# Lennart0HU/Master-Thesis-Deep-Reinforcement-Learning-DDPG-in-Home-Energy-Management

Hardware: NVIDIA B200
Metric: shems_LU1 env-steps/s (batched) (higher is better)
Workload: dtype f32/f64 mixed (Julia promotion rules)

## Files before the change

include/shems_b200.h:

```cpp
#ifndef SHEMS_B200_H
#define SHEMS_B200_H

#include <stdint.h>

#ifdef __cplusplus
extern "C" {
#endif

#define SHEMS_API __attribute__((visibility("default")))

enum {
  SHEMS_OK = 0,
  SHEMS_ERR_INVALID = -1,
  SHEMS_ERR_CUDA = -2,
  SHEMS_ERR_BOUNDS = -3,
  SHEMS_ERR_KEY = -4,
  SHEMS_ERR_STATE = -5
};

SHEMS_API const char* shems_last_error(void);
SHEMS_API int32_t shems_version(void);
SHEMS_API int64_t shems_env_kernel_launches(void);
SHEMS_API int32_t shems_device_count(void);

#define SHEMS_STATE_SIZE 9
#define SHEMS_ACTION_SIZE 2
#define SHEMS_TRACE_COLS 23
#define SHEMS_SERIES_COLS 8

enum {
  SHEMS_S_SOC_B = 0, SHEMS_S_SOC_EV, SHEMS_S_C_EV, SHEMS_S_D_E, SHEMS_S_G_E,
  SHEMS_S_P_BUY, SHEMS_S_H_COS, SHEMS_S_H_SIN, SHEMS_S_SEASON
};

enum {
  SHEMS_COL_SOC_EV = 0,
  SHEMS_COL_H_COUNTDOWN,
  SHEMS_COL_ELECTKWH,
  SHEMS_COL_PV_GENERATION,
  SHEMS_COL_P_BUY,
  SHEMS_COL_HOUR_COS,
  SHEMS_COL_HOUR_SIN,
  SHEMS_COL_SEASON
};

enum {
  SHEMS_T_INDEX = 0, SHEMS_T_C_EV, SHEMS_T_EV_TARGET, SHEMS_T_EV, SHEMS_T_SOC_EV,
  SHEMS_T_REWARD, SHEMS_T_PROFIT, SHEMS_T_DISCOMFORT, SHEMS_T_PENALTY, SHEMS_T_PV_DE,
  SHEMS_T_B_DE, SHEMS_T_GR_DE, SHEMS_T_PV_B, SHEMS_T_PV_GR, SHEMS_T_PV_EV, SHEMS_T_B_EV,
  SHEMS_T_GR_EV, SHEMS_T_EX_EV, SHEMS_T_GR_B, SHEMS_T_B_GR, SHEMS_T_B, SHEMS_T_B_TARGET,
  SHEMS_T_SOC_B
};

typedef struct ShemsParams {
  float pv_eta;
  float b_eta;
  float b_soc_min;
  float b_soc_max;
  double b_rate_max;
  float b_loss;
  float ev_soc_min;
  float ev_soc_max;
  float ev_rate_max;
  float penalty_weight;
  double sell_discount;
  double discomfort_weight_ev;
  double disc_pot;
  double penalty_weight_f64;
  int32_t penalty_in_f64;
  int32_t reward_form;
} ShemsParams;

SHEMS_API int32_t shems_params_for_charger(int32_t charger_id, ShemsParams* out);
enum { SHEMS_ENV_LU1 = 0, SHEMS_ENV_LU7 = 1, SHEMS_ENV_LU1_INPUT0607 = 2 };
SHEMS_API int32_t shems_params_for_env(int32_t env_variant, int32_t charger_id, ShemsParams* out);

SHEMS_API int32_t shems_series_from_csv(const char* path, float* series_out, int32_t capacity, int32_t* nrows_out);

typedef struct ShemsEnv ShemsEnv;

SHEMS_API int32_t shems_create(const ShemsParams* params, const float* series_host,
                               int32_t nrows, int32_t maxsteps, int64_t n_envs,
                               int32_t device, ShemsEnv** out);
SHEMS_API int32_t shems_create_groups(const ShemsParams* params, int32_t n_groups, const int64_t* group_sizes, const float* series_host,
                                      int32_t series_per_group, int32_t nrows, int32_t maxsteps, int32_t device, ShemsEnv** out);
SHEMS_API int32_t shems_destroy(ShemsEnv* env);
SHEMS_API int32_t shems_set_stream(ShemsEnv* env, void* cuda_stream);
SHEMS_API int32_t shems_sync(ShemsEnv* env);

enum { SHEMS_RESET_DETERMINISTIC = 0, SHEMS_RESET_HOST_DRAWS = 1, SHEMS_RESET_DEVICE_PHILOX = 2 };
SHEMS_API int32_t shems_reset(ShemsEnv* env, int32_t mode, const int32_t* idx0_host,
                              const float* socb0_host, uint64_t seed, int64_t env_id_base);

SHEMS_API int32_t shems_step(ShemsEnv* env, const float* act_dev, int32_t track,
                             float* reward_dev, double* reward64_dev, float* obs_dev, double* trace_dev);

SHEMS_API int32_t shems_action_rule(ShemsEnv* env, float* bev_dev);
SHEMS_API int32_t shems_action_drl(ShemsEnv* env, const float* target_dev, float* bev_dev);
SHEMS_API int32_t shems_finished(const ShemsEnv* env, int32_t* out);

SHEMS_API int32_t shems_state_ptr(ShemsEnv* env, float** obs_dev , int32_t** idx_dev );
SHEMS_API int32_t shems_get_state(ShemsEnv* env, float* obs_host , int32_t* idx_host );
SHEMS_API int32_t shems_set_state(ShemsEnv* env, const float* obs_host , const int32_t* idx_host );
SHEMS_API int32_t shems_get_step(const ShemsEnv* env, int32_t* step);
SHEMS_API int64_t shems_num_envs(const ShemsEnv* env);
// ... 135 lines not shown
```

master-thesis-deep-reinforcement-learning-ddpg-in-home-energy-management_b200/_lib.py:

```python
import ctypes as C
import os

HERE = os.path.dirname(os.path.abspath(__file__))
LIB_PATH = os.environ.get("SHEMS_B200_LIB", os.path.join(HERE, "libshems_b200.so"))

OK, ERR_INVALID, ERR_CUDA, ERR_BOUNDS, ERR_KEY, ERR_STATE = 0, -1, -2, -3, -4, -5
RESET_DETERMINISTIC, RESET_HOST_DRAWS, RESET_DEVICE_PHILOX = 0, 1, 2
POLICY_RULE, POLICY_RANDOM, POLICY_TAPE = 0, 1, 2
ENV_LU1, ENV_LU7, ENV_LU1_INPUT0607 = 0, 1, 2
NET_ACTOR, NET_CRITIC, NET_ACTOR_TARGET, NET_CRITIC_TARGET, NET_ACTOR_BEST = 0, 1, 2, 3, 4
DP_HANDLE_BYTES = 192


class ShemsParams(C.Structure):
    _fields_ = [
        ("pv_eta", C.c_float), ("b_eta", C.c_float), ("b_soc_min", C.c_float), ("b_soc_max", C.c_float),
        ("b_rate_max", C.c_double), ("b_loss", C.c_float), ("ev_soc_min", C.c_float), ("ev_soc_max", C.c_float),
        ("ev_rate_max", C.c_float), ("penalty_weight", C.c_float), ("sell_discount", C.c_double),
        ("discomfort_weight_ev", C.c_double), ("disc_pot", C.c_double),
        ("penalty_weight_f64", C.c_double), ("penalty_in_f64", C.c_int32), ("reward_form", C.c_int32),
    ]


class DdpgParams(C.Structure):
    _fields_ = [
        ("state_size", C.c_int32), ("action_size", C.c_int32), ("l1", C.c_int32), ("l2", C.c_int32),
        ("batch", C.c_int32), ("gamma", C.c_float), ("tau", C.c_float), ("lr_actor", C.c_float),
        ("lr_critic", C.c_float), ("adam_beta1", C.c_double), ("adam_beta2", C.c_double), ("adam_eps", C.c_double),
        ("act_lo", C.c_float * 2), ("act_hi", C.c_float * 2), ("use_tensor_cores", C.c_int32), ("population", C.c_int32),
    ]


class ShemsRolloutArgs(C.Structure):
    _fields_ = [
        ("policy", C.c_int32), ("n_steps", C.c_int32), ("seed", C.c_uint64), ("env_id_base", C.c_int64),
        ("tape_dev", C.c_void_p), ("ep_return_dev", C.c_void_p), ("replay", C.c_void_p), ("trace_dev", C.c_void_p),
        ("obs_traj_dev", C.c_void_p), ("reward_traj_dev", C.c_void_p), ("tape_unscaled", C.c_int32),
    ]


EXPLOIT_MAX_GROUPS = 16


class DdpgExploitParams(C.Structure):
    _fields_ = [
        ("frac", C.c_double), ("factor_lo", C.c_float), ("factor_hi", C.c_float), ("keys", C.c_int32), ("round", C.c_uint32),
        ("seed", C.c_uint64), ("n_groups", C.c_int32), ("group_start", C.c_int32 * (EXPLOIT_MAX_GROUPS + 1)),
    ]


class ShemsError(RuntimeError):
    def __init__(self, code, msg):
        super().__init__(f"[{code}] {msg}")
        self.code = code


class ShemsBoundsError(ShemsError, IndexError):
    """Julia BoundsError of next_state! (shems_LU1.jl:266-268)."""


class ShemsKeyError(ShemsError, KeyError):
    """Julia KeyError of capacities[charger_id] (shems_LU1.jl:95)."""


VP, PF, PI, PD = C.c_void_p, C.POINTER(C.c_float), C.POINTER(C.c_int32), C.POINTER(C.c_double)
I32, I64, U64, F32 = C.c_int32, C.c_int64, C.c_uint64, C.c_float

SIGNATURES = {
    "shems_last_error": (C.c_char_p, []),
    "shems_version": (I32, []),
    "shems_device_count": (I32, []),
    "shems_env_kernel_launches": (I64, []),
    "shems_params_for_charger": (I32, [I32, C.POINTER(ShemsParams)]),
    "shems_params_for_env": (I32, [I32, I32, C.POINTER(ShemsParams)]),
    "shems_series_from_csv": (I32, [C.c_char_p, PF, I32, PI]),
    "shems_create": (I32, [C.POINTER(ShemsParams), PF, I32, I32, I64, I32, C.POINTER(VP)]),
    "shems_create_groups": (I32, [C.POINTER(ShemsParams), I32, C.POINTER(I64), PF, I32, I32, I32, I32, C.POINTER(VP)]),
    "shems_destroy": (I32, [VP]),
    "shems_set_stream": (I32, [VP, VP]),
    "shems_sync": (I32, [VP]),
    "shems_reset": (I32, [VP, I32, PI, PF, U64, I64]),
    "shems_step": (I32, [VP, VP, I32, VP, VP, VP, VP]),
    "shems_action_rule": (I32, [VP, VP]),
    "shems_action_drl": (I32, [VP, VP, VP]),
    "shems_finished": (I32, [VP, PI]),
    "shems_state_ptr": (I32, [VP, C.POINTER(VP), C.POINTER(VP)]),
    "shems_get_state": (I32, [VP, PF, PI]),
    "shems_set_state": (I32, [VP, PF, PI]),
    "shems_get_step": (I32, [VP, PI]),
    "shems_num_envs": (I64, [VP]),
    "shems_num_rows": (I32, [VP]),
    "shems_rollout": (I32, [VP, C.POINTER(ShemsRolloutArgs)]),
    "replay_create": (I32, [I64, I32, C.POINTER(VP)]),
    "replay_destroy": (I32, [VP]),
    "replay_set_stream": (I32, [VP, VP]),
    "replay_length": (I64, [VP]),
    "replay_capacity": (I64, [VP]),
    "replay_series_count": (I32, [VP]),
    "replay_push": (I32, [VP, VP, VP, VP, VP, VP, I64]),
    "replay_push_groups": (I32, [C.POINTER(VP), I32, VP, VP, VP, VP, VP, I64]),
    "replay_sample": (I32, [VP, I32, PI, U64, VP, VP, VP, VP, VP]),
    "replay_minmax": (I32, [VP, I64, PI, U64, PF, PF]),
    "replay_get": (I32, [VP, PF, PF, PF, PF, PF]),
    "ddpg_default_params": (I32, [C.POINTER(DdpgParams)]),
    "ddpg_create": (I32, [C.POINTER(DdpgParams), I32, C.POINTER(VP)]),
    "ddpg_destroy": (I32, [VP]),
    "ddpg_set_stream": (I32, [VP, VP]),
    "ddpg_sync": (I32, [VP]),
    "ddpg_set_fused": (I32, [VP, I32]),
    "ddpg_init": (I32, [VP, U64]),
    "ddpg_set_layer": (I32, [VP, I32, I32, PF, PF]),
    "ddpg_get_layer": (I32, [VP, I32, I32, PF, PF]),
    "ddpg_get_grad": (I32, [VP, I32, I32, PF, PF]),
    "ddpg_num_params": (I64, [VP, I32]),
    "ddpg_set_norm": (I32, [VP, PF, PF]),
    "ddpg_act": (I32, [VP, VP, I64, F32, U64, I64, I64, VP, VP, VP]),
    "ddpg_act_soa": (I32, [VP, VP, I64, F32, U64, I64, I64, VP, VP, VP]),
    "ddpg_act_ou": (I32, [VP, VP, I64, F32, F32, F32, F32, VP, U64, I64, I64, VP, VP, VP]),
    "ddpg_set_noise": (I32, [VP, I32, F32, F32, F32]),
    "ddpg_episode": (I32, [VP, VP, C.POINTER(VP), I32, I32, F32, U64, I32, I64, VP, VP]),
    "ddpg_update": (I32, [VP, VP, I32, PI, U64]),
    "ddpg_update_phase": (I32, [VP, VP, I32, PI, U64, F32]),
    "ddpg_update_batch": (I32, [VP, VP, VP, VP, VP, VP]),
    "ddpg_dp_export": (I32, [VP, VP]),
    "ddpg_dp_connect": (I32, [VP, I32, I32, VP]),
    "ddpg_dp_prepare": (I32, [VP, I64]),
    "ddpg_update_dp": (I32, [VP, VP, I32, PI, U64]),
    "ddpg_dp_status": (I32, [VP, PI]),
    "ddpg_get_losses": (I32, [VP, PF, PF]),
    "ddpg_select_learner": (I32, [VP, I32]),
    "ddpg_population": (I32, [VP]),
    "ddpg_update_population": (I32, [VP, C.POINTER(VP), I32, PI, C.POINTER(U64)]),
    "ddpg_set_hparams": (I32, [VP, F32, F32, F32, F32, F32]),
    "ddpg_get_hparams": (I32, [VP, PF, PF, PF, PF, PF]),
    "shems_tc_gemm": (I32, [VP, I64, I32, VP, I64, I32, VP, I64, I32, I32, I32, I32, VP, VP, I64, I32, VP, VP]),
    "ddpg_grad_buffer": (I32, [VP, C.POINTER(VP), C.POINTER(I64)]),
    "ddpg_rollout": (I32, [VP, VP, I32, F32, U64, I64, VP, VP, VP]),
    "ddpg_evaluate": (I32, [VP, VP, I32, I32, I64, VP, VP, VP]),
    "ddpg_keep_best": (I32, [VP, VP, I64, I32, VP]),
    "ddpg_get_best": (I32, [VP, PD, PI]),
    "ddpg_set_best": (I32, [VP, PD, PI]),
    "ddpg_exploit": (I32, [VP, VP, C.POINTER(DdpgExploitParams), VP]),
    "ddpg_state_floats": (I64, [VP]),
    "ddpg_get_state": (I32, [VP, PF, PD]),
    "ddpg_set_state": (I32, [VP, PF, PD]),
    "ddpg_get_ou_state": (I32, [VP, PF, C.POINTER(I64)]),
    "ddpg_set_ou_state": (I32, [VP, PF, I64]),
}

_lib = None


def lib():
    global _lib
    if _lib is None:
# ... 46 lines not shown
```

master-thesis-deep-reinforcement-learning-ddpg-in-home-energy-management_b200/csrc/common.h:

```cpp
#pragma once
#include <cuda_runtime.h>
#include <stdint.h>
#include <stdio.h>
#include <stdarg.h>
#include "../../include/shems_b200.h"
#include "ring.cuh"

void shems_set_error(const char* fmt, ...);

#define CUDA_TRY(expr)                                                                     \
  do {                                                                                     \
    cudaError_t _e = (expr);                                                               \
    if (_e != cudaSuccess) {                                                               \
      shems_set_error("%s:%d %s -> %s", __FILE__, __LINE__, #expr, cudaGetErrorString(_e)); \
      return SHEMS_ERR_CUDA;                                                               \
    }                                                                                      \
  } while (0)

#define REQUIRE(cond, code, ...)  \
  do {                            \
    if (!(cond)) {                \
      shems_set_error(__VA_ARGS__); \
      return (code);              \
    }                             \
  } while (0)

struct DeviceGuard {
  int prev = -1;
  bool ok = true;
  explicit DeviceGuard(int dev) {
    if (cudaGetDevice(&prev) != cudaSuccess) { ok = false; return; }
    if (prev != dev && cudaSetDevice(dev) != cudaSuccess) ok = false;
  }
  ~DeviceGuard() { if (prev >= 0) cudaSetDevice(prev); }
};
#define GUARD(dev)                                             \
  DeviceGuard _guard(dev);                                     \
  if (!_guard.ok) {                                            \
    cudaError_t _e = cudaGetLastError();                       \
    shems_set_error("cannot select CUDA device %d: %s", (dev), cudaGetErrorString(_e)); \
    return SHEMS_ERR_CUDA;                                     \
  }

struct DevParams {
  float pv_eta, b_eta, smin, smax, loss, evmin, evmax, evR, pw;
  float one_m_l;
  float one_m_l_e;
  float C;
  float span;
  float R_f;
  float R_dn, R_up;
  float smax95_up;
  double R, sell, dw, pot;
  double pw_d;
  int pen_f64, reward_form;
  int reward_mode;
  double eta_d, one_m_l_d, C_d, smax95;
  float r_eta_f, r_span_f;
  double r_eta_d, r_C_d;
  int fast_eta_f, fast_span_f;
  int fast_d;
  double span_d, r_span_d;
  int fast_all;
};

#define SHEMS_MAX_GROUPS 16

struct RingSeries {
  unsigned long long env_serial;
  int series;
  int nrows;
  float* rows;
};

struct ShemsReplay {
  int device;
  cudaStream_t stream;
  int64_t capacity, length, head;
  float* alloc;
  float* ring;
  int32_t* idx_scratch;
  int64_t idx_scratch_n;
  float* minmax_scratch;
  void* group_refs; int group_refs_n;
  RingSeries src[RING_MAX_SERIES];
  const float* src_ptrs[RING_MAX_SERIES];
  int n_src;
};

struct ShemsEnv {
  int device;
  cudaStream_t stream;
  DevParams dp;
  ShemsParams params;
  int32_t nrows, maxsteps;
  int64_t n;
  float4* series;
  float* obs;
  int32_t* idx;
  int32_t* d_maxidx;
  int32_t max_idx;
  int32_t* h_maxidx;
  cudaEvent_t ev_maxidx; bool max_pending;
  int32_t step;
  unsigned long long serial;
  bool was_reset;
  bool consistent;
  int32_t* scratch_i; float* scratch_f;
  int n_groups;
  DevParams gdp[SHEMS_MAX_GROUPS];
  float4* gseries[SHEMS_MAX_GROUPS];
  long long gstart[SHEMS_MAX_GROUPS + 1];
};

int replay_after_rollout(ShemsReplay* rp, int64_t n_written);
int replay_series_entry(ShemsReplay* rp, unsigned long long serial, int series, const float4* rows_dev, int nrows, cudaStream_t user,
                        int* entry);
int32_t ensure_rows(ShemsEnv* e, int64_t need);
```

master-thesis-deep-reinforcement-learning-ddpg-in-home-energy-management_b200/csrc/env.cu:

```cuda
#include <new>
#include <vector>
#include <string.h>
#include <math.h>
#include <stdlib.h>

#include "common.h"
#include "philox.cuh"
#include "shems_device.cuh"

static thread_local char g_err[512] = "";
void shems_set_error(const char* fmt, ...) {
  va_list ap;
  va_start(ap, fmt);
  vsnprintf(g_err, sizeof(g_err), fmt, ap);
  va_end(ap);
}
extern "C" const char* shems_last_error(void) { return g_err; }
extern "C" int32_t shems_version(void) { return 200; }
static long long g_env_launches = 0;
extern "C" int64_t shems_env_kernel_launches(void) { return __atomic_load_n(&g_env_launches, __ATOMIC_RELAXED); }
#define COUNT_LAUNCH() __atomic_add_fetch(&g_env_launches, 1, __ATOMIC_RELAXED)
extern "C" int32_t shems_device_count(void) {
  int n = 0;
  if (cudaGetDeviceCount(&n) != cudaSuccess) { cudaGetLastError(); return 0; }
// ... 371 lines not shown
                          const float* __restrict__ tape, int tape_unscaled, RolloutSinks S, long long n0, long long n1, int lockstep) {
  const long long n = n0 + (long long)blockIdx.x * blockDim.x + threadIdx.x;
  if (n >= n1) return;
  int idx = idx_arr[n];
  float Soc_b = obs[0 * N + n], Soc_ev = obs[1 * N + n];
  float c_ev, d_e, g_e, p_buy;
  { const Row8 r = load_row(series, idx); c_ev = r.cd; d_e = r.d_e; g_e = r.g_e; p_buy = r.p_buy; }
  double ret = 0.0;
  RingWalk ring{};
  if (S.ring) { long long slot = S.head + n; if (slot >= S.cap) slot -= S.cap; ring = ring_walk(S.ring, slot, N, S.cap); }
  const uint64_t id = (uint64_t)(env_id_base + n);
  auto step = [&](auto cls, int t, uint32_t w0, uint32_t w1) {
    constexpr int CLS = decltype(cls)::value;
    StepIn s;
    s.Soc_b = Soc_b; s.Soc_ev = Soc_ev; s.c_ev = c_ev; s.d_e = d_e; s.g_e = g_e; s.p_buy = p_buy;
    float B, EV, Bt, EVt, a_raw0, a_raw1;
    bool track_neg = false;
    if (POLICY == SHEMS_POLICY_RULE) {
      shems_action_rule<true>(P, s.Soc_b, s.Soc_ev, s.d_e, s.g_e, B, EV);
      Bt = 0.0f; EVt = 0.0f; a_raw0 = B; a_raw1 = EV; track_neg = true;
    } else {
      if (POLICY == SHEMS_POLICY_RANDOM) {
        a_raw0 = action_from_word(w0);
        a_raw1 = action_from_word(w1);
        Bt = (a_raw0 + 1.0f) * 0.5f;
        EVt = (a_raw1 + 1.0f) * 0.5f;
      } else {
        Bt = tape[((size_t)t * 2 + 0) * N + n];
        EVt = tape[((size_t)t * 2 + 1) * N + n];
        a_raw0 = Bt; a_raw1 = EVt;
        if (tape_unscaled) {
          Bt = (float)(((double)a_raw0 + 1.0) * 0.5);
          EVt = (float)(((double)a_raw1 + 1.0) * 0.5);
        }
      }
      shems_action_drl<true, CLS>(P, s.Soc_b, s.Soc_ev, s.c_ev, s.d_e, s.g_e, Bt, EVt, B, EV);
    }
    StepTrace tr;
    const StepOut o = shems_flows<false, true, CLS>(P, s, B, EV, EVt, track_neg, &tr);
    const Row8 nx = load_row(series, idx + 1);
    float Soc_ev_new = o.Soc_ev;
    if (nx.cd >= 0.0f && (CLS == ROW_ANY ? c_ev == -1.0f : row_noev<CLS>)) Soc_ev_new = nx.soc_ev;
    if (S.ring) {
      ring_store_compact(ring.q, Soc_b, Soc_ev, a_raw0, a_raw1, (float)o.reward, o.Soc_b, Soc_ev_new, S.src_entry, idx);
      ring_walk_next(ring);
    }
    if (S.reward_traj) S.reward_traj[(size_t)t * N + n] = (float)o.reward;
    Soc_b = o.Soc_b; Soc_ev = Soc_ev_new; c_ev = nx.cd; d_e = nx.d_e; g_e = nx.g_e; p_buy = nx.p_buy;
    idx += 1;
    ret += o.reward;
  };
  const unsigned mask = __activemask();
  if (lockstep && __all_sync(mask, idx == __shfl_sync(mask, idx, __ffs(mask) - 1))) {
    uint32_t rw[4] = {0u, 0u, 0u, 0u};
    for (int t = 0; t < T; ++t) {
      if (POLICY == SHEMS_POLICY_RANDOM) {
        const unsigned st_abs = (unsigned)(step0 + t);
        if ((st_abs & 1u) == 0u || t == 0) philox4x32_10(K, id, st_abs >> 1, STREAM_ACTION, rw);
        if (st_abs & 1u) { rw[0] = rw[2]; rw[1] = rw[3]; }
      }
      switch (row_class(P, c_ev, d_e, g_e)) {
        case ROW_A_NOEV: step(RowTag<ROW_A_NOEV>{}, t, rw[0], rw[1]); break;
        case ROW_B_NOEV: step(RowTag<ROW_B_NOEV>{}, t, rw[0], rw[1]); break;
        case ROW_A_EV: step(RowTag<ROW_A_EV>{}, t, rw[0], rw[1]); break;
        case ROW_B_EV: step(RowTag<ROW_B_EV>{}, t, rw[0], rw[1]); break;
        default: step(RowTag<ROW_ANY>{}, t, rw[0], rw[1]); break;
      }
    }
  } else {
    for (int t = POLICY == SHEMS_POLICY_RANDOM ? -(step0 & 1) : 0; t < T; t += 2) {
      uint32_t rw[4] = {0u, 0u, 0u, 0u};
      if (POLICY == SHEMS_POLICY_RANDOM) philox4x32_10(K, id, (unsigned)(step0 + t) >> 1, STREAM_ACTION, rw);
      if (t >= 0) step(RowTag<ROW_ANY>{}, t, rw[0], rw[1]);
      if (t + 1 < T) step(RowTag<ROW_ANY>{}, t + 1, rw[2], rw[3]);
    }
  }
  const Row8 r = load_row(series, idx);
  obs[0 * N + n] = Soc_b; obs[1 * N + n] = Soc_ev; obs[2 * N + n] = r.cd; obs[3 * N + n] = r.d_e; obs[4 * N + n] = r.g_e;
  obs[5 * N + n] = r.p_buy; obs[6 * N + n] = r.h_cos; obs[7 * N + n] = r.h_sin; obs[8 * N + n] = r.season;
  idx_arr[n] = idx;
  if (S.ep_return) S.ep_return[n] = ret;
}

static inline unsigned grid_for(long long n, int block) { return (unsigned)((n + block - 1) / block); }

static int rollout_min_blocks(int device, long long n, bool compact, bool lean) {
  static int forced = -1;
  if (forced < 0) { const char* ev = getenv("SHEMS_ROLLOUT_MIN_BLOCKS"); forced = ev ? atoi(ev) : 0; }
  if (forced == 6 || forced == 7 || forced == 8) return forced;
  if (compact) return lean ? 7 : 6;
  static int sms[64];
  if (device >= 0 && device < 64 && sms[device] == 0) {
    int v = 0;
    if (cudaDeviceGetAttribute(&v, cudaDevAttrMultiProcessorCount, device) != cudaSuccess || v <= 0) { cudaGetLastError(); v = 148; }
    sms[device] = v;
  }
  const int nsm = (device >= 0 && device < 64) ? sms[device] : 148;
  const double ctas = (double)((n + ROLLOUT_THREADS - 1) / ROLLOUT_THREADS);
  int best = ROLLOUT_MIN_BLOCKS; double best_cost = 1e300;
  for (int b = 6; b <= 8; ++b) {
    const double waves = ctas / ((double)nsm * b);
    const double full = floor(waves), frac = waves - full;
    const double last = frac > 0.0 ? (frac < 0.45 ? 0.45 : frac) : 0.0;
    const double penalty = b == 6 ? 1.0 : (b == 7 ? 1.015 : 1.03);
    const double cost = (full + last) * b * penalty;
    if (cost < best_cost - 1e-9) { best_cost = cost; best = b; }
  }
  return best;
}

static bool ring_compact_enabled() {
  const char* ev = getenv("SHEMS_RING_COMPACT");
  return !(ev && atoi(ev) == 0);
}

static bool rollout_lean_enabled() {
  const char* ev = getenv("SHEMS_ROLLOUT_LEAN");
  return !(ev && atoi(ev) == 0);
}

static bool rollout_lockstep_enabled() {
  const char* ev = getenv("SHEMS_ROLLOUT_LOCKSTEP");
  return !(ev && atoi(ev) == 0);
}

extern "C" int32_t shems_create_groups(const ShemsParams* params, int32_t n_groups, const int64_t* group_sizes, const float* series_host,
                                       int32_t series_per_group, int32_t nrows, int32_t maxsteps, int32_t device, ShemsEnv** out) {
  REQUIRE(params && series_host && out && group_sizes, SHEMS_ERR_INVALID, "shems_create: NULL argument");
  REQUIRE(n_groups >= 1 && n_groups <= SHEMS_MAX_GROUPS, SHEMS_ERR_INVALID, "shems_create: n_groups=%d (1..%d)", n_groups, SHEMS_MAX_GROUPS);
  int64_t n_envs = 0;
  for (int g = 0; g < n_groups; ++g) {
    REQUIRE(group_sizes[g] >= 1, SHEMS_ERR_INVALID, "shems_create: group_sizes[%d]=%lld", g, (long long)group_sizes[g]);
    n_envs += group_sizes[g];
  }
  REQUIRE(nrows >= 2 && maxsteps >= 1, SHEMS_ERR_INVALID, "shems_create: nrows=%d maxsteps=%d", nrows, maxsteps);
  REQUIRE(nrows - maxsteps >= 1, SHEMS_ERR_INVALID,
          "shems_create: nrows - maxsteps = %d < 1: rand(1:(nrow-maxsteps)) would be empty (shems_LU1.jl:225)", nrows - maxsteps);
  REQUIRE(shems_device_count() > 0, SHEMS_ERR_CUDA, "shems_create: no CUDA device (this library has no CPU fallback)");
  GUARD(device);
  ShemsEnv* e = new (std::nothrow) ShemsEnv();
  REQUIRE(e, SHEMS_ERR_INVALID, "shems_create: out of host memory");
  memset(e, 0, sizeof(*e));
  e->device = device; e->stream = 0; e->params = params[0]; e->dp = make_dev_params(params[0]);
  e->nrows = nrows; e->maxsteps = maxsteps; e->n = n_envs; e->max_idx = 1; e->consistent = true;
  e->n_groups = n_groups;
  static unsigned long long next_serial = 0;
  e->serial = __atomic_add_fetch(&next_serial, 1, __ATOMIC_RELAXED);
  const int n_series = series_per_group ? n_groups : 1;
  std::vector<float> rows((size_t)n_series * nrows * 8);
  for (int g = 0; g < n_series; ++g)
    for (int r = 0; r < nrows; ++r)
      for (int c = 0; c < 8; ++c) rows[((size_t)g * nrows + r) * 8 + c] = series_host[((size_t)g * 8 + c) * nrows + r];
  cudaError_t st = cudaSuccess;
  if ((st = cudaMalloc(&e->series, sizeof(float) * rows.size())) != cudaSuccess ||
      (st = cudaMalloc(&e->obs, sizeof(float) * 9 * (size_t)n_envs)) != cudaSuccess ||
      (st = cudaMalloc(&e->idx, sizeof(int32_t) * (size_t)n_envs)) != cudaSuccess ||
      (st = cudaMalloc(&e->d_maxidx, sizeof(int32_t))) != cudaSuccess ||
      (st = cudaMemcpy(e->series, rows.data(), sizeof(float) * rows.size(), cudaMemcpyHostToDevice)) != cudaSuccess ||
      (st = cudaMemset(e->obs, 0, sizeof(float) * 9 * (size_t)n_envs)) != cudaSuccess ||
      (st = cudaMemset(e->idx, 0, sizeof(int32_t) * (size_t)n_envs)) != cudaSuccess) {
    shems_set_error("shems_create: %s", cudaGetErrorString(st));
    shems_destroy(e);
    return SHEMS_ERR_CUDA;
  }
  if ((st = cudaMallocHost((void**)&e->h_maxidx, sizeof(int32_t))) != cudaSuccess ||
      (st = cudaEventCreateWithFlags(&e->ev_maxidx, cudaEventDisableTiming)) != cudaSuccess) {
    shems_set_error("shems_create: %s", cudaGetErrorString(st));
    shems_destroy(e);
    return SHEMS_ERR_CUDA;
  }
  for (int g = 0; g < n_groups; ++g) {
    e->gdp[g] = make_dev_params(params[g]);
    e->gseries[g] = e->series + (series_per_group ? (size_t)g * nrows * 2 : 0);
    e->gstart[g + 1] = e->gstart[g] + group_sizes[g];
  }
  *out = e;
  return SHEMS_OK;
}

extern "C" int32_t shems_create(const ShemsParams* params, const float* series_host, int32_t nrows, int32_t maxsteps,
                                int64_t n_envs, int32_t device, ShemsEnv** out) {
  REQUIRE(n_envs >= 1, SHEMS_ERR_INVALID, "shems_create: n_envs=%lld", (long long)n_envs);
  return shems_create_groups(params, 1, &n_envs, series_host, 0, nrows, maxsteps, device, out);
}

extern "C" int32_t shems_destroy(ShemsEnv* e) {
  if (!e) return SHEMS_OK;
  GUARD(e->device);
  cudaFree(e->series); cudaFree(e->obs); cudaFree(e->idx); cudaFree(e->d_maxidx); cudaFree(e->scratch_i); cudaFree(e->scratch_f);
  if (e->h_maxidx) cudaFreeHost(e->h_maxidx);
  if (e->ev_maxidx) cudaEventDestroy(e->ev_maxidx);
  delete e;
  return SHEMS_OK;
}

extern "C" int32_t shems_set_stream(ShemsEnv* e, void* s) {
  REQUIRE(e, SHEMS_ERR_INVALID, "shems_set_stream: NULL handle");
  e->stream = (cudaStream_t)s;
  return SHEMS_OK;
}
extern "C" int32_t shems_sync(ShemsEnv* e) {
  REQUIRE(e, SHEMS_ERR_INVALID, "shems_sync: NULL handle");
  GUARD(e->device);
  CUDA_TRY(cudaStreamSynchronize(e->stream));
  return SHEMS_OK;
}
extern "C" int64_t shems_num_envs(const ShemsEnv* e) { return e ? e->n : 0; }
extern "C" int32_t shems_num_rows(const ShemsEnv* e) { return e ? e->nrows : 0; }
extern "C" int32_t shems_get_step(const ShemsEnv* e, int32_t* step) {
  REQUIRE(e && step, SHEMS_ERR_INVALID, "shems_get_step: NULL argument");
  *step = e->step;
  return SHEMS_OK;
}
extern "C" int32_t shems_finished(const ShemsEnv* e, int32_t* out) {
  REQUIRE(e && out, SHEMS_ERR_INVALID, "shems_finished: NULL argument");
  *out = 0;
  return SHEMS_OK;
}

int32_t ensure_rows(ShemsEnv* e, int64_t need) {
  if ((int64_t)e->max_idx + need <= e->nrows) return 0;
  if (e->max_pending) {
    cudaEventSynchronize(e->ev_maxidx);
    e->max_idx = *e->h_maxidx + e->step;
    e->max_pending = false;
    if ((int64_t)e->max_idx + need <= e->nrows) return 0;
  }
  return e->max_idx;
}

extern "C" int32_t shems_reset(ShemsEnv* e, int32_t mode, const int32_t* idx0_host, const float* socb0_host, uint64_t seed,
                               int64_t env_id_base) {
  REQUIRE(e, SHEMS_ERR_INVALID, "shems_reset: NULL handle");
  REQUIRE(mode >= 0 && mode <= 2, SHEMS_ERR_INVALID, "shems_reset: unknown mode %d", mode);
  GUARD(e->device);
  const int hi = e->nrows - e->maxsteps;
  if (mode == SHEMS_RESET_HOST_DRAWS) {
    REQUIRE(idx0_host && socb0_host, SHEMS_ERR_INVALID, "shems_reset: HOST_DRAWS needs idx0_host and socb0_host");
    for (int64_t i = 0; i < e->n; ++i)
      REQUIRE(idx0_host[i] >= 1 && idx0_host[i] <= hi, SHEMS_ERR_INVALID, "shems_reset: idx0[%lld]=%d outside 1..%d", (long long)i,
              idx0_host[i], hi);
    if (!e->scratch_i) {
      CUDA_TRY(cudaMalloc(&e->scratch_i, sizeof(int32_t) * (size_t)e->n));
      CUDA_TRY(cudaMalloc(&e->scratch_f, sizeof(float) * (size_t)e->n));
    }
    CUDA_TRY(cudaMemcpyAsync(e->scratch_i, idx0_host, sizeof(int32_t) * (size_t)e->n, cudaMemcpyHostToDevice, e->stream));
    CUDA_TRY(cudaMemcpyAsync(e->scratch_f, socb0_host, sizeof(float) * (size_t)e->n, cudaMemcpyHostToDevice, e->stream));
  }
  CUDA_TRY(cudaMemsetAsync(e->d_maxidx, 0, sizeof(int32_t), e->stream));
  for (int g = 0; g < e->n_groups; ++g) {
    const long long n0 = e->gstart[g], n1 = e->gstart[g + 1];
    COUNT_LAUNCH();
    shems_reset_kernel<<<grid_for(n1 - n0, 256), 256, 0, e->stream>>>(e->gdp[g], e->gseries[g], e->nrows, e->maxsteps, e->n, mode, e->scratch_i,
                                                                     e->scratch_f, seed, env_id_base, e->obs, e->idx, e->d_maxidx, n0, n1);
  }
  CUDA_TRY(cudaGetLastError());
  if (mode == SHEMS_RESET_DETERMINISTIC) { e->max_idx = 1; e->max_pending = false; }
  else {
    CUDA_TRY(cudaMemcpyAsync(e->h_maxidx, e->d_maxidx, sizeof(int32_t), cudaMemcpyDeviceToHost, e->stream));
    CUDA_TRY(cudaEventRecord(e->ev_maxidx, e->stream));
    e->max_idx = hi; e->max_pending = true;
  }
  e->step = 0;
  e->was_reset = true;
  e->consistent = true;
  return SHEMS_OK;
}

extern "C" int32_t shems_step(ShemsEnv* e, const float* act_dev, int32_t track, float* reward_dev, double* reward64_dev, float* obs_dev,
                              double* trace_dev) {
  REQUIRE(e && act_dev, SHEMS_ERR_INVALID, "shems_step: NULL argument");
  REQUIRE(e->was_reset, SHEMS_ERR_STATE, "shems_step: reset! (or shems_set_state) must come first");
  if (ensure_rows(e, 1)) {
    shems_set_error("BoundsError: attempt to access %d-row series at row %d (next_state!, shems_LU1.jl:266-268)", e->nrows, e->max_idx + 1);
    return SHEMS_ERR_BOUNDS;
  }
  GUARD(e->device);
  const int tn = track < 0 ? 1 : 0;
#define LAUNCH_STEP(FS, TR)                                                                                                             \
  COUNT_LAUNCH();                                                                                                                       \
  if (!TR && e->gdp[g].fast_all)                                                                                                        \
    shems_step_kernel<FS, false, true><<<grid_for(n1 - n0, STEP_THREADS), STEP_THREADS, 0, e->stream>>>(                                   \
        e->gdp[g], e->gseries[g], e->n, e->obs, e->idx, act_dev, tn, reward_dev, reward64_dev, obs_dev, trace_dev, n0, n1);              \
  else                                                                                                                                  \
    shems_step_kernel<FS, TR, false><<<grid_for(n1 - n0, STEP_THREADS), STEP_THREADS, 0, e->stream>>>(                                     \
        e->gdp[g], e->gseries[g], e->n, e->obs, e->idx, act_dev, tn, reward_dev, reward64_dev, obs_dev, trace_dev, n0, n1)
  for (int g = 0; g < e->n_groups; ++g) {
    const long long n0 = e->gstart[g], n1 = e->gstart[g + 1];
    if (e->consistent) { if (trace_dev) { LAUNCH_STEP(true, true); } else { LAUNCH_STEP(true, false); } }
    else { if (trace_dev) { LAUNCH_STEP(false, true); } else { LAUNCH_STEP(false, false); } }
  }
#undef LAUNCH_STEP
  CUDA_TRY(cudaGetLastError());
  e->max_idx += 1;
  e->step += 1;
  e->consistent = true;
  return SHEMS_OK;
}

extern "C" int32_t shems_action_rule(ShemsEnv* e, float* bev_dev) {
  REQUIRE(e && bev_dev, SHEMS_ERR_INVALID, "shems_action_rule: NULL argument");
  GUARD(e->device);
  for (int g = 0; g < e->n_groups; ++g, COUNT_LAUNCH())
    shems_action_kernel<true><<<grid_for(e->gstart[g + 1] - e->gstart[g], 256), 256, 0, e->stream>>>(e->gdp[g], e->n, e->obs, nullptr, bev_dev,
                                                                                                    e->gstart[g], e->gstart[g + 1]);
  CUDA_TRY(cudaGetLastError());
  return SHEMS_OK;
}
extern "C" int32_t shems_action_drl(ShemsEnv* e, const float* target_dev, float* bev_dev) {
  REQUIRE(e && target_dev && bev_dev, SHEMS_ERR_INVALID, "shems_action_drl: NULL argument");
  GUARD(e->device);
  for (int g = 0; g < e->n_groups; ++g, COUNT_LAUNCH())
    shems_action_kernel<false><<<grid_for(e->gstart[g + 1] - e->gstart[g], 256), 256, 0, e->stream>>>(e->gdp[g], e->n, e->obs, target_dev, bev_dev,
                                                                                                     e->gstart[g], e->gstart[g + 1]);
  CUDA_TRY(cudaGetLastError());
  return SHEMS_OK;
}

extern "C" int32_t shems_state_ptr(ShemsEnv* e, float** obs_dev, int32_t** idx_dev) {
  REQUIRE(e, SHEMS_ERR_INVALID, "shems_state_ptr: NULL handle");
  if (obs_dev) *obs_dev = e->obs;
  if (idx_dev) *idx_dev = e->idx;
  return SHEMS_OK;
}
extern "C" int32_t shems_get_state(ShemsEnv* e, float* obs_host, int32_t* idx_host) {
  REQUIRE(e && obs_host, SHEMS_ERR_INVALID, "shems_get_state: NULL argument");
  GUARD(e->device);
  CUDA_TRY(cudaMemcpyAsync(obs_host, e->obs, sizeof(float) * 9 * (size_t)e->n, cudaMemcpyDeviceToHost, e->stream));
  if (idx_host) CUDA_TRY(cudaMemcpyAsync(idx_host, e->idx, sizeof(int32_t) * (size_t)e->n, cudaMemcpyDeviceToHost, e->stream));
  CUDA_TRY(cudaStreamSynchronize(e->stream));
  return SHEMS_OK;
}
extern "C" int32_t shems_set_state(ShemsEnv* e, const float* obs_host, const int32_t* idx_host) {
  REQUIRE(e && obs_host && idx_host, SHEMS_ERR_INVALID, "shems_set_state: NULL argument");
  GUARD(e->device);
  int32_t mx = 1;
  for (int64_t i = 0; i < e->n; ++i) {
    REQUIRE(idx_host[i] >= 1 && idx_host[i] <= e->nrows, SHEMS_ERR_INVALID, "shems_set_state: idx[%lld]=%d outside 1..%d", (long long)i,
            idx_host[i], e->nrows);
    mx = idx_host[i] > mx ? idx_host[i] : mx;
  }
  CUDA_TRY(cudaMemcpyAsync(e->obs, obs_host, sizeof(float) * 9 * (size_t)e->n, cudaMemcpyHostToDevice, e->stream));
  CUDA_TRY(cudaMemcpyAsync(e->idx, idx_host, sizeof(int32_t) * (size_t)e->n, cudaMemcpyHostToDevice, e->stream));
  CUDA_TRY(cudaStreamSynchronize(e->stream));
  e->max_idx = mx; e->max_pending = false;
  e->was_reset = true;
  e->consistent = false;
  return SHEMS_OK;
}

extern "C" int32_t shems_rollout(ShemsEnv* e, const ShemsRolloutArgs* a) {
  REQUIRE(e && a, SHEMS_ERR_INVALID, "shems_rollout: NULL argument");
  REQUIRE(e->was_reset, SHEMS_ERR_STATE, "shems_rollout: reset! must come first");
  REQUIRE(a->n_steps >= 1, SHEMS_ERR_INVALID, "shems_rollout: n_steps=%d", a->n_steps);
  REQUIRE(a->policy >= 0 && a->policy <= 2, SHEMS_ERR_INVALID, "shems_rollout: unknown policy %d", a->policy);
  REQUIRE(a->policy != SHEMS_POLICY_TAPE || a->tape_dev, SHEMS_ERR_INVALID, "shems_rollout: POLICY_TAPE needs tape_dev");
  REQUIRE(!(a->policy == SHEMS_POLICY_TAPE && a->replay && !a->tape_unscaled), SHEMS_ERR_INVALID,
          "shems_rollout: POLICY_TAPE with a replay sink needs tape_unscaled = 1 (actions in [-1,1], as remember() stores them)");
  if (ensure_rows(e, a->n_steps)) {
    shems_set_error("BoundsError: rollout of %d steps from row %d leaves the %d-row series (next_state!, shems_LU1.jl:266-268)", a->n_steps,
                    e->max_idx, e->nrows);
    return SHEMS_ERR_BOUNDS;
  }
  GUARD(e->device);
  RolloutSinks S;
  memset(&S, 0, sizeof(S));
  S.ep_return = a->ep_return_dev; S.trace = a->trace_dev; S.obs_traj = a->obs_traj_dev; S.reward_traj = a->reward_traj_dev;
  S.cap = 1;
  const int64_t total = (int64_t)a->n_steps * e->n;
  if (a->replay) {
    ShemsReplay* rp = a->replay;
    REQUIRE(rp->device == e->device, SHEMS_ERR_INVALID, "shems_rollout: replay lives on device %d, env on %d", rp->device, e->device);
    REQUIRE(total <= rp->capacity || rp->capacity % e->n == 0, SHEMS_ERR_INVALID,
            "shems_rollout: replay capacity %lld must hold n_steps*n_envs=%lld or be a multiple of n_envs=%lld", (long long)rp->capacity,
            (long long)total, (long long)e->n);
    REQUIRE(e->n <= rp->capacity, SHEMS_ERR_INVALID, "shems_rollout: replay capacity %lld < n_envs %lld", (long long)rp->capacity, (long long)e->n);
    S.ring = rp->ring; S.cap = rp->capacity; S.head = rp->head;
  }
#define LAUNCH_RO_F(POL, TR, MB, FA, CO)                                                                                            \
  shems_rollout_kernel<POL, TR, MB, FA, CO><<<grid_for(n1 - n0, ROLLOUT_THREADS), ROLLOUT_THREADS, 0, e->stream>>>(                      \
      e->gdp[g], e->gseries[g], e->n, e->obs, e->idx, a->n_steps, e->step, a->seed, a->env_id_base, a->tape_dev, a->tape_unscaled, S, n0, n1)
#define LAUNCH_RO_C(POL, TR, MB, FA)                                                                                                \
  do { if (compact) LAUNCH_RO_F(POL, TR, MB, FA, true); else LAUNCH_RO_F(POL, TR, MB, FA, false); } while (0)
#define LAUNCH_RO(POL, TR, MB)                                                                                                      \
  do { if (!TR && e->gdp[g].fast_all) LAUNCH_RO_C(POL, false, MB, true); else LAUNCH_RO_C(POL, TR, MB, false); } while (0)
#define LAUNCH_RO_MB(POL)                                                                                                           \
  do {                                                                                                                              \
    if (tr) LAUNCH_RO(POL, true, ROLLOUT_MIN_BLOCKS);                                                                               \
    else if (mb == 7) LAUNCH_RO(POL, false, 7);                                                                                     \
    else if (mb == 8) LAUNCH_RO(POL, false, 8);                                                                                     \
    else LAUNCH_RO(POL, false, ROLLOUT_MIN_BLOCKS);                                                                                 \
  } while (0)
#define LAUNCH_LEAN(POL, MB)                                                                                                        \
  shems_rollout_lean_kernel<POL, MB><<<grid_for(n1 - n0, ROLLOUT_THREADS), ROLLOUT_THREADS, 0, e->stream>>>(                           \
      e->gdp[g], e->gseries[g], e->n, e->obs, e->idx, a->n_steps, e->step, keys, a->env_id_base, a->tape_dev, a->tape_unscaled, S, n0, n1, \
      lockstep)
#define LAUNCH_LEAN_MB(POL)                                                                                                         \
  do {                                                                                                                              \
    if (mb == 7) LAUNCH_LEAN(POL, 7);                                                                                               \
    else if (mb == 8) LAUNCH_LEAN(POL, 8);                                                                                          \
    else LAUNCH_LEAN(POL, ROLLOUT_MIN_BLOCKS);                                                                                      \
  } while (0)
  const bool tr = a->trace_dev != nullptr;
  const bool may_lean = !tr && !a->obs_traj_dev && e->consistent && rollout_lean_enabled();
  const PhiloxKeys keys = philox_keys(a->seed);
  const int lockstep = rollout_lockstep_enabled() ? 1 : 0;
  const bool may_compact = a->replay && e->consistent && e->nrows <= RING_TAG_MAX_ROW && ring_compact_enabled();
  for (int g = 0; g < e->n_groups; ++g) {
    const long long n0 = e->gstart[g], n1 = e->gstart[g + 1];
    bool compact = false;
    if (may_compact) {
      int entry;
      const int series = (int)((e->gseries[g] - e->series) / (2 * (size_t)e->nrows));
      const int st = replay_series_entry(a->replay, e->serial, series, e->gseries[g], e->nrows, e->stream, &entry);
      if (st) return st;
      compact = entry >= 0;
      S.src_entry = compact ? ring_tag(entry, 0) : 0u;
    }
    const bool lean = may_lean && e->gdp[g].fast_all && (!a->replay || (compact && e->n % 32 == 0 && S.cap % 32 == 0));
    const int mb = rollout_min_blocks(e->device, n1 - n0, compact, lean);
    COUNT_LAUNCH();
    if (lean) {
      switch (a->policy) {
        case SHEMS_POLICY_RULE: LAUNCH_LEAN_MB(SHEMS_POLICY_RULE); break;
        case SHEMS_POLICY_RANDOM: LAUNCH_LEAN_MB(SHEMS_POLICY_RANDOM); break;
        default: LAUNCH_LEAN_MB(SHEMS_POLICY_TAPE); break;
      }
      continue;
    }
    switch (a->policy) {
      case SHEMS_POLICY_RULE: LAUNCH_RO_MB(SHEMS_POLICY_RULE); break;
      case SHEMS_POLICY_RANDOM: LAUNCH_RO_MB(SHEMS_POLICY_RANDOM); break;
      default: LAUNCH_RO_MB(SHEMS_POLICY_TAPE); break;
    }
  }
#undef LAUNCH_LEAN_MB
#undef LAUNCH_LEAN
#undef LAUNCH_RO_MB
#undef LAUNCH_RO
#undef LAUNCH_RO_C
#undef LAUNCH_RO_F
  CUDA_TRY(cudaGetLastError());
  e->max_idx += a->n_steps;
  e->step += a->n_steps;
  e->consistent = true;
  if (a->replay) return replay_after_rollout(a->replay, total);
  return SHEMS_OK;
}
```

master-thesis-deep-reinforcement-learning-ddpg-in-home-energy-management_b200/csrc/ring.cuh:

```cuda
#pragma once
#include <stddef.h>
#include <stdint.h>
#include <string.h>

#include "philox.cuh"

#define RING_FIELDS 23
#define RING_S 0
#define RING_A 9
#define RING_R 11
#define RING_S2 12
#define RING_DONE 21
#define RING_SRC 22
#define RING_TRANSITION_FIELDS 22
__host__ __device__ __forceinline__ size_t ring_base(long long slot) { return ((size_t)(slot >> 5) * RING_FIELDS) * 32 + (size_t)(slot & 31); }

#define RING_MAX_SERIES 16
#define RING_HEADER_FLOATS 32
#define RING_TAG_ROW_BITS 24
#define RING_TAG_ROW_MASK ((1u << RING_TAG_ROW_BITS) - 1u)
#define RING_TAG_MAX_ROW ((int32_t)RING_TAG_ROW_MASK)
static_assert(RING_MAX_SERIES * sizeof(float*) <= RING_HEADER_FLOATS * sizeof(float), "the series table fits the header");

__host__ __device__ __forceinline__ size_t ring_alloc_floats(long long cap) {
  return RING_HEADER_FLOATS + RING_FIELDS * 32 * (((size_t)cap + 31) / 32);
}
__host__ __device__ __forceinline__ float* ring_in_alloc(float* alloc) { return alloc + RING_HEADER_FLOATS; }
__host__ __device__ __forceinline__ const float* const* ring_table(const float* ring) {
  return reinterpret_cast<const float* const*>(ring - RING_HEADER_FLOATS);
}

__host__ __device__ __forceinline__ uint32_t ring_tag(int entry, int row1) { return ((uint32_t)entry << RING_TAG_ROW_BITS) | (uint32_t)row1; }
__host__ __device__ __forceinline__ const float* ring_row(const float* const* table, const float* q) {
#ifdef __CUDA_ARCH__
  const uint32_t tag = __float_as_uint(q[RING_SRC * 32]);
#else
  uint32_t tag;
  memcpy(&tag, q + RING_SRC * 32, sizeof(tag));
#endif
  return tag ? table[tag >> RING_TAG_ROW_BITS] + 8 * (size_t)((tag & RING_TAG_ROW_MASK) - 1u) : nullptr;
}
__host__ __device__ __forceinline__ float ring_field(const float* q, const float* row, int f) {
  if (row) {
    if (f >= RING_S + 2 && f < RING_A) return row[f - RING_S - 1];
    if (f >= RING_S2 + 2 && f < RING_DONE) return row[8 + f - RING_S2 - 1];
    if (f == RING_DONE) return 0.0f;
  }
  return q[f * 32];
}

__host__ __device__ __forceinline__ long long ring_slot(long long li, long long head, long long len, long long cap) {
  long long slot = head - len + li;
  if (slot < 0) slot += cap;
  return slot;
}
__host__ __device__ __forceinline__ long long ring_push_slot(long long head, long long i, long long cap) {
  const long long slot = head + i;
  return slot - (slot / cap) * cap;
}

struct RingWalk {
  float* q;
  const float* last;
  ptrdiff_t stride, back;
};
__host__ __device__ __forceinline__ RingWalk ring_walk(float* ring, long long slot, long long N, long long cap) {
  RingWalk w;
  w.q = ring + ring_base(slot);
  w.stride = (ptrdiff_t)(N >> 5) * RING_FIELDS * 32;
  w.back = w.stride - (ptrdiff_t)(cap >> 5) * RING_FIELDS * 32;
  w.last = ring - w.back;
  return w;
}
__host__ __device__ __forceinline__ void ring_walk_next(RingWalk& w) { w.q += (w.q >= w.last) ? w.back : w.stride; }

__host__ __device__ __forceinline__ long long ring_draw(uint64_t seed, uint64_t j, uint32_t update, long long len) {
  uint32_t w[4];
  philox4x32_10(seed, j, update, STREAM_SAMPLE, w);
  long long li = (long long)(u53(w[0], w[1]) * (double)len);
  if (li >= len) li = len - 1;
  return li;
}

__device__ __forceinline__ void ring_store_own(float* q, float sb, float sev, float a0, float a1, float r, float sb2, float sev2) {
  q[(RING_S + 0) * 32] = sb; q[(RING_S + 1) * 32] = sev;
  q[(RING_A + 0) * 32] = a0; q[(RING_A + 1) * 32] = a1;
  q[RING_R * 32] = r;
  q[(RING_S2 + 0) * 32] = sb2; q[(RING_S2 + 1) * 32] = sev2;
}
__device__ __forceinline__ void ring_store_full(float* q, const float* s, float a0, float a1, float r, const float* s2, float done) {
  ring_store_own(q, s[0], s[1], a0, a1, r, s2[0], s2[1]);
#pragma unroll
  for (int k = 2; k < 9; ++k) q[(RING_S + k) * 32] = s[k];
#pragma unroll
  for (int k = 2; k < 9; ++k) q[(RING_S2 + k) * 32] = s2[k];
  q[RING_DONE * 32] = done;
  q[RING_SRC * 32] = 0.0f;
}
__device__ __forceinline__ void ring_store_compact(float* q, float sb, float sev, float a0, float a1, float r, float sb2, float sev2,
                                                   uint32_t series_tag, int row) {
  ring_store_own(q, sb, sev, a0, a1, r, sb2, sev2);
  q[RING_SRC * 32] = __uint_as_float(series_tag | (uint32_t)row);
}
```

Baseline: 124.3 billion.

## Add paired-env rollout kernel sharing series row loads when all envs align

Adds a rollout kernel in which each thread steps two adjacent environments. They share one series-row load and row-class dispatch per step, and replay-ring writes use float2 stores. It is enabled by default when every env starts at the same row (uniform_row), the group is lean, sizes are even, and the grid still fills enough SMs at a lower min-blocks bound. This cuts series loads and issue overhead per env-step, but halves thread-level parallelism and may raise register pressure.

New measurement: 137.0 billion, median of 6. 10.2% higher.

```diff
diff --git a/include/shems_b200.h b/include/shems_b200.h
--- a/include/shems_b200.h
+++ b/include/shems_b200.h
@@ -21,6 +21,7 @@
 SHEMS_API const char* shems_last_error(void);
 SHEMS_API int32_t shems_version(void);
 SHEMS_API int64_t shems_env_kernel_launches(void);
+SHEMS_API int64_t shems_rollout_pair_launches(void);
 SHEMS_API int32_t shems_device_count(void);
 
 #define SHEMS_STATE_SIZE 9
diff --git a/master-thesis-deep-reinforcement-learning-ddpg-in-home-energy-management_b200/_lib.py b/master-thesis-deep-reinforcement-learning-ddpg-in-home-energy-management_b200/_lib.py
--- a/master-thesis-deep-reinforcement-learning-ddpg-in-home-energy-management_b200/_lib.py
+++ b/master-thesis-deep-reinforcement-learning-ddpg-in-home-energy-management_b200/_lib.py
@@ -71,6 +71,7 @@
     "shems_version": (I32, []),
     "shems_device_count": (I32, []),
     "shems_env_kernel_launches": (I64, []),
+    "shems_rollout_pair_launches": (I64, []),
     "shems_params_for_charger": (I32, [I32, C.POINTER(ShemsParams)]),
     "shems_params_for_env": (I32, [I32, I32, C.POINTER(ShemsParams)]),
     "shems_series_from_csv": (I32, [C.c_char_p, PF, I32, PI]),
diff --git a/master-thesis-deep-reinforcement-learning-ddpg-in-home-energy-management_b200/csrc/common.h b/master-thesis-deep-reinforcement-learning-ddpg-in-home-energy-management_b200/csrc/common.h
--- a/master-thesis-deep-reinforcement-learning-ddpg-in-home-energy-management_b200/csrc/common.h
+++ b/master-thesis-deep-reinforcement-learning-ddpg-in-home-energy-management_b200/csrc/common.h
@@ -106,6 +106,7 @@
   unsigned long long serial;
   bool was_reset;
   bool consistent;
+  bool uniform_row;
   int32_t* scratch_i; float* scratch_f;
   int n_groups;
   DevParams gdp[SHEMS_MAX_GROUPS];
diff --git a/master-thesis-deep-reinforcement-learning-ddpg-in-home-energy-management_b200/csrc/env.cu b/master-thesis-deep-reinforcement-learning-ddpg-in-home-energy-management_b200/csrc/env.cu
--- a/master-thesis-deep-reinforcement-learning-ddpg-in-home-energy-management_b200/csrc/env.cu
+++ b/master-thesis-deep-reinforcement-learning-ddpg-in-home-energy-management_b200/csrc/env.cu
@@ -477,20 +477,117 @@
   if (S.ep_return) S.ep_return[n] = ret;
 }
 
+template <int POLICY, int MINB>
+__global__ void __launch_bounds__(ROLLOUT_THREADS, MINB)
+shems_rollout_pair_kernel(DevParams P, const float4* __restrict__ series, long long N, float* __restrict__ obs,
+                          int32_t* __restrict__ idx_arr, int T, int step0, PhiloxKeys K, long long env_id_base,
+                          const float* __restrict__ tape, int tape_unscaled, RolloutSinks S, long long n0, long long n1) {
+  const long long n = n0 + 2 * ((long long)blockIdx.x * blockDim.x + threadIdx.x);
+  if (n >= n1) return;
+  int idx = idx_arr[n];
+  float Soc_b[2] = {obs[n], obs[n + 1]}, Soc_ev[2] = {obs[N + n], obs[N + n + 1]};
+  float c_ev, d_e, g_e, p_buy;
+  { const Row8 r = load_row(series, idx); c_ev = r.cd; d_e = r.d_e; g_e = r.g_e; p_buy = r.p_buy; }
+  double ret[2] = {0.0, 0.0};
+  RingWalk ring{};
+  if (S.ring) { long long slot = S.head + n; if (slot >= S.cap) slot -= S.cap; ring = ring_walk(S.ring, slot, N, S.cap); }
+  const uint64_t id = (uint64_t)(env_id_base + n);
+  auto step = [&](auto cls, int t, const uint32_t (&rw)[2][4]) {
+    constexpr int CLS = decltype(cls)::value;
+    const Row8 nx = load_row(series, idx + 1);
+    float a_raw0[2], a_raw1[2], r32[2], Soc_b2[2], Soc_ev2[2];
+#pragma unroll
+    for (int i = 0; i < 2; ++i) {
+      StepIn s;
+      s.Soc_b = Soc_b[i]; s.Soc_ev = Soc_ev[i]; s.c_ev = c_ev; s.d_e = d_e; s.g_e = g_e; s.p_buy = p_buy;
+      float B, EV, Bt, EVt;
+      bool track_neg = false;
+      if (POLICY == SHEMS_POLICY_RULE) {
+        shems_action_rule<true>(P, s.Soc_b, s.Soc_ev, s.d_e, s.g_e, B, EV);
+        Bt = 0.0f; EVt = 0.0f; a_raw0[i] = B; a_raw1[i] = EV; track_neg = true;
+      } else {
+        if (POLICY == SHEMS_POLICY_RANDOM) {
+          a_raw0[i] = action_from_word(rw[i][0]);
+          a_raw1[i] = action_from_word(rw[i][1]);
+          Bt = (a_raw0[i] + 1.0f) * 0.5f;
+          EVt = (a_raw1[i] + 1.0f) * 0.5f;
+        } else {
+          Bt = tape[((size_t)t * 2 + 0) * N + n + i];
+          EVt = tape[((size_t)t * 2 + 1) * N + n + i];
+          a_raw0[i] = Bt; a_raw1[i] = EVt;
+          if (tape_unscaled) {
+            Bt = (float)(((double)a_raw0[i] + 1.0) * 0.5);
+            EVt = (float)(((double)a_raw1[i] + 1.0) * 0.5);
+          }
+        }
+        shems_action_drl<true, CLS>(P, s.Soc_b, s.Soc_ev, s.c_ev, s.d_e, s.g_e, Bt, EVt, B, EV);
+      }
+      StepTrace tr;
+      const StepOut o = shems_flows<false, true, CLS>(P, s, B, EV, EVt, track_neg, &tr);
+      Soc_ev2[i] = (nx.cd >= 0.0f && (CLS == ROW_ANY ? c_ev == -1.0f : row_noev<CLS>)) ? nx.soc_ev : o.Soc_ev;
+      Soc_b2[i] = o.Soc_b;
+      r32[i] = (float)o.reward;
+      ret[i] += o.reward;
+    }
+    if (S.ring) {
+      ring_store_compact_pair(ring.q, Soc_b, Soc_ev, a_raw0, a_raw1, r32, Soc_b2, Soc_ev2, S.src_entry, idx);
+      ring_walk_next(ring);
+    }
+    if (S.reward_traj) { S.reward_traj[(size_t)t * N + n] = r32[0]; S.reward_traj[(size_t)t * N + n + 1] = r32[1]; }
+#pragma unroll
+    for (int i = 0; i < 2; ++i) { Soc_b[i] = Soc_b2[i]; Soc_ev[i] = Soc_ev2[i]; }
+    c_ev = nx.cd; d_e = nx.d_e; g_e = nx.g_e; p_buy = nx.p_buy;
+    idx += 1;
+  };
+  uint32_t rw[2][4] = {};
+  for (int t = 0; t < T; ++t) {
+    if (POLICY == SHEMS_POLICY_RANDOM) {
+      const unsigned st_abs = (unsigned)(step0 + t);
+      if ((st_abs & 1u) == 0u || t == 0) {
+        philox4x32_10(K, id, st_abs >> 1, STREAM_ACTION, rw[0]);
+        philox4x32_10(K, id + 1, st_abs >> 1, STREAM_ACTION, rw[1]);
+      }
+      if (st_abs & 1u) {
+#pragma unroll
+        for (int i = 0; i < 2; ++i) { rw[i][0] = rw[i][2]; rw[i][1] = rw[i][3]; }
+      }
+    }
+    switch (row_class(P, c_ev, d_e, g_e)) {
+      case ROW_A_NOEV: step(RowTag<ROW_A_NOEV>{}, t, rw); break;
+      case ROW_B_NOEV: step(RowTag<ROW_B_NOEV>{}, t, rw); break;
+      case ROW_A_EV: step(RowTag<ROW_A_EV>{}, t, rw); break;
+      case ROW_B_EV: step(RowTag<ROW_B_EV>{}, t, rw); break;
+      default: step(RowTag<ROW_ANY>{}, t, rw); break;
+    }
+  }
+  const Row8 r = load_row(series, idx);
+#pragma unroll
+  for (int i = 0; i < 2; ++i) {
+    const long long m = n + i;
+    obs[0 * N + m] = Soc_b[i]; obs[1 * N + m] = Soc_ev[i]; obs[2 * N + m] = r.cd; obs[3 * N + m] = r.d_e; obs[4 * N + m] = r.g_e;
+    obs[5 * N + m] = r.p_buy; obs[6 * N + m] = r.h_cos; obs[7 * N + m] = r.h_sin; obs[8 * N + m] = r.season;
+    idx_arr[m] = idx;
+    if (S.ep_return) S.ep_return[m] = ret[i];
+  }
+}
+
 static inline unsigned grid_for(long long n, int block) { return (unsigned)((n + block - 1) / block); }
 
+static int sm_count(int device) {
+  static int sms[64];
+  if (device >= 0 && device < 64 && sms[device] == 0) {
+    int v = 0;
+    if (cudaDeviceGetAttribute(&v, cudaDevAttrMultiProcessorCount, device) != cudaSuccess || v <= 0) { cudaGetLastError(); v = 148; }
+    sms[device] = v;
+  }
+  return (device >= 0 && device < 64) ? sms[device] : 148;
+}
 static int rollout_min_blocks(int device, long long n, bool compact, bool lean) {
   static int forced = -1;
   if (forced < 0) { const char* ev = getenv("SHEMS_ROLLOUT_MIN_BLOCKS"); forced = ev ? atoi(ev) : 0; }
   if (forced == 6 || forced == 7 || forced == 8) return forced;
   if (compact) return lean ? 7 : 6;
-  static int sms[64];
-  if (device >= 0 && device < 64 && sms[device] == 0) {
-    int v = 0;
-    if (cudaDeviceGetAttribute(&v, cudaDevAttrMultiProcessorCount, device) != cudaSuccess || v <= 0) { cudaGetLastError(); v = 148; }
-    sms[device] = v;
-  }
-  const int nsm = (device >= 0 && device < 64) ? sms[device] : 148;
+  const int nsm = sm_count(device);
   const double ctas = (double)((n + ROLLOUT_THREADS - 1) / ROLLOUT_THREADS);
   int best = ROLLOUT_MIN_BLOCKS; double best_cost = 1e300;
   for (int b = 6; b <= 8; ++b) {
@@ -518,6 +615,24 @@
   const char* ev = getenv("SHEMS_ROLLOUT_LOCKSTEP");
   return !(ev && atoi(ev) == 0);
 }
+
+#ifndef ROLLOUT_PAIR_MIN_BLOCKS
+#define ROLLOUT_PAIR_MIN_BLOCKS 4
+#endif
+#ifndef ROLLOUT_PAIR_MIN_WAVES
+#define ROLLOUT_PAIR_MIN_WAVES 1
+#endif
+static int rollout_pair_mode() {
+  const char* ev = getenv("SHEMS_ROLLOUT_PAIR");
+  return ev ? atoi(ev) : 1;
+}
+static bool rollout_pair_fills(int device, long long n, int mode) {
+  if (mode == 2) return true;
+  const long long ctas = (n / 2 + ROLLOUT_THREADS - 1) / ROLLOUT_THREADS;
+  return ctas >= (long long)ROLLOUT_PAIR_MIN_WAVES * sm_count(device) * ROLLOUT_PAIR_MIN_BLOCKS;
+}
+static long long g_pair_launches = 0;
+extern "C" int64_t shems_rollout_pair_launches(void) { return __atomic_load_n(&g_pair_launches, __ATOMIC_RELAXED); }
 
 extern "C" int32_t shems_create_groups(const ShemsParams* params, int32_t n_groups, const int64_t* group_sizes, const float* series_host,
                                        int32_t series_per_group, int32_t nrows, int32_t maxsteps, int32_t device, ShemsEnv** out) {
@@ -659,6 +774,11 @@
   e->step = 0;
   e->was_reset = true;
   e->consistent = true;
+  e->uniform_row = mode == SHEMS_RESET_DETERMINISTIC || hi == 1;
+  if (mode == SHEMS_RESET_HOST_DRAWS) {
+    e->uniform_row = true;
+    for (int64_t i = 1; i < e->n && e->uniform_row; ++i) e->uniform_row = idx0_host[i] == idx0_host[0];
+  }
   return SHEMS_OK;
 }
 
@@ -741,6 +861,8 @@
   e->max_idx = mx; e->max_pending = false;
   e->was_reset = true;
   e->consistent = false;
+  e->uniform_row = true;
+  for (int64_t i = 1; i < e->n && e->uniform_row; ++i) e->uniform_row = idx_host[i] == idx_host[0];
   return SHEMS_OK;
 }
 
@@ -790,6 +912,9 @@
   shems_rollout_lean_kernel<POL, MB><<<grid_for(n1 - n0, ROLLOUT_THREADS), ROLLOUT_THREADS, 0, e->stream>>>(                           \
       e->gdp[g], e->gseries[g], e->n, e->obs, e->idx, a->n_steps, e->step, keys, a->env_id_base, a->tape_dev, a->tape_unscaled, S, n0, n1, \
       lockstep)
+#define LAUNCH_PAIR(POL)                                                                                                            \
+  shems_rollout_pair_kernel<POL, ROLLOUT_PAIR_MIN_BLOCKS><<<grid_for((n1 - n0) / 2, ROLLOUT_THREADS), ROLLOUT_THREADS, 0, e->stream>>>( \
+      e->gdp[g], e->gseries[g], e->n, e->obs, e->idx, a->n_steps, e->step, keys, a->env_id_base, a->tape_dev, a->tape_unscaled, S, n0, n1)
 #define LAUNCH_LEAN_MB(POL)                                                                                                         \
   do {                                                                                                                              \
     if (mb == 7) LAUNCH_LEAN(POL, 7);                                                                                               \
@@ -800,6 +925,7 @@
   const bool may_lean = !tr && !a->obs_traj_dev && e->consistent && rollout_lean_enabled();
   const PhiloxKeys keys = philox_keys(a->seed);
   const int lockstep = rollout_lockstep_enabled() ? 1 : 0;
+  const int pair_mode = lockstep ? rollout_pair_mode() : 0;
   const bool may_compact = a->replay && e->consistent && e->nrows <= RING_TAG_MAX_ROW && ring_compact_enabled();
   for (int g = 0; g < e->n_groups; ++g) {
     const long long n0 = e->gstart[g], n1 = e->gstart[g + 1];
@@ -813,8 +939,19 @@
       S.src_entry = compact ? ring_tag(entry, 0) : 0u;
     }
     const bool lean = may_lean && e->gdp[g].fast_all && (!a->replay || (compact && e->n % 32 == 0 && S.cap % 32 == 0));
+    const bool pair = lean && e->uniform_row && pair_mode != 0 && (n1 - n0) % 2 == 0 && (!a->replay || (S.head + n0) % 2 == 0) &&
+                      rollout_pair_fills(e->device, n1 - n0, pair_mode);
     const int mb = rollout_min_blocks(e->device, n1 - n0, compact, lean);
     COUNT_LAUNCH();
+    if (pair) {
+      __atomic_add_fetch(&g_pair_launches, 1, __ATOMIC_RELAXED);
+      switch (a->policy) {
+        case SHEMS_POLICY_RULE: LAUNCH_PAIR(SHEMS_POLICY_RULE); break;
+        case SHEMS_POLICY_RANDOM: LAUNCH_PAIR(SHEMS_POLICY_RANDOM); break;
+        default: LAUNCH_PAIR(SHEMS_POLICY_TAPE); break;
+      }
+      continue;
+    }
     if (lean) {
       switch (a->policy) {
         case SHEMS_POLICY_RULE: LAUNCH_LEAN_MB(SHEMS_POLICY_RULE); break;
@@ -830,6 +967,7 @@
     }
   }
 #undef LAUNCH_LEAN_MB
+#undef LAUNCH_PAIR
 #undef LAUNCH_LEAN
 #undef LAUNCH_RO_MB
 #undef LAUNCH_RO
diff --git a/master-thesis-deep-reinforcement-learning-ddpg-in-home-energy-management_b200/csrc/ring.cuh b/master-thesis-deep-reinforcement-learning-ddpg-in-home-energy-management_b200/csrc/ring.cuh
--- a/master-thesis-deep-reinforcement-learning-ddpg-in-home-energy-management_b200/csrc/ring.cuh
+++ b/master-thesis-deep-reinforcement-learning-ddpg-in-home-energy-management_b200/csrc/ring.cuh
@@ -102,3 +102,13 @@
   ring_store_own(q, sb, sev, a0, a1, r, sb2, sev2);
   q[RING_SRC * 32] = __uint_as_float(series_tag | (uint32_t)row);
 }
+__device__ __forceinline__ void ring_store_compact_pair(float* q, const float sb[2], const float sev[2], const float a0[2], const float a1[2],
+                                                        const float r[2], const float sb2[2], const float sev2[2], uint32_t series_tag, int row) {
+  auto st2 = [q](int f, float x, float y) { *reinterpret_cast<float2*>(q + f * 32) = make_float2(x, y); };
+  st2(RING_S + 0, sb[0], sb[1]); st2(RING_S + 1, sev[0], sev[1]);
+  st2(RING_A + 0, a0[0], a0[1]); st2(RING_A + 1, a1[0], a1[1]);
+  st2(RING_R, r[0], r[1]);
+  st2(RING_S2 + 0, sb2[0], sb2[1]); st2(RING_S2 + 1, sev2[0], sev2[1]);
+  const float tag = __uint_as_float(series_tag | (uint32_t)row);
+  st2(RING_SRC, tag, tag);
+}
```
